# vqdang/hover_net

Measured on AMD Instinct MI355X. Metric: tiles/sec (270x270, batch 32) end-to-end incl. watershed, higher is better.
Workload: dtype fp32

## Files before the change

hover_net_amd/csrc/hvn_api.hip:

```cpp
#include <hip/hip_runtime.h>
#include <stdio.h>
#include <string.h>

#include <vector>

#include "../../include/hvn.h"
#include "hvn_kernels.h"

static thread_local char g_err[512] = "";

static int fail(int code, const char *fmt, const char *a = "", long b = 0)
{
    snprintf(g_err, sizeof(g_err), fmt, a, b);
    return code;
}

extern "C" {

int hvn_version(void) { return 104; }

#ifndef HVN_BUILD_ID
#define HVN_BUILD_ID "unstamped"
#endif
static const char hvn_build_tag[] = "hvn-build-id:" HVN_BUILD_ID;
// ... 71 lines not shown
        a.is_f32 = op->x_dtype;
        a.H = op->x.h; a.W = op->x.w;
        a.w = op->w; a.bias = op->bias;
        a.y = (float *)op->y.base;
        a.ysn = op->y.sn; a.ysy = op->y.sy; a.ysx = op->y.sx;
        a.N = batch; a.Ho = op->y.h; a.Wo = op->y.w; a.pad = op->pad_t; a.relu = op->relu; a.out_bf16 = op->act_dtype == 1;
        if (op->kh != 7 || op->kw != 7 || op->x.c != 3 || op->y.c != 64 || !op->w || !op->bias)
            return fail(HVN_E_ARG, "conv0: expects 7x7x3->64 with bias%s", "");
        if (!aligned16(a.y) || (a.ysx & 3) || (a.ysy & 3) || (a.ysn & 3)) return fail(HVN_E_ARG, "conv0: output view not 16-byte aligned%s", "");
        return hvn_launch_conv0(a, s);
    }
    case HVN_OP_CONV: {
        ConvArgs a;
        memset(&a, 0, sizeof(a));
        a.x = (const float *)op->x.base;
        a.xsn = op->x.sn; a.xsy = op->x.sy; a.xsx = op->x.sx;
        a.H = op->x.h; a.W = op->x.w; a.Cin = op->x.c;
        a.w = op->w; a.bias = op->bias;
        a.pre_s = op->pre_scale; a.pre_b = op->pre_shift;
        a.post_s = op->post_scale; a.post_b = op->post_shift;
        a.res = (const float *)op->res.base;
        a.rsn = op->res.sn; a.rsy = op->res.sy; a.rsx = op->res.sx;
        a.y = (float *)op->y.base;
        a.ysn = op->y.sn; a.ysy = op->y.sy; a.ysx = op->y.sx;
        a.N = batch; a.Ho = op->y.h; a.Wo = op->y.w; a.Cout = op->cout;
        a.KH = op->kh; a.KW = op->kw; a.stride = op->stride; a.pad_t = op->pad_t; a.pad_l = op->pad_l;
        a.relu = op->relu;
        a.groups = op->groups > 1 ? op->groups : 1;
        a.x2 = (const float *)op->x2.base;
        a.x2sn = op->x2.sn; a.x2sy = op->x2.sy; a.x2sx = op->x2.sx;
        a.Cin2 = a.x2 ? op->x2.c : 0;
        a.stride2 = op->_rsv > 0 ? op->_rsv : 1;
        if (a.x2 && (op->kh != 1 || op->kw != 1 || a.stride != 1 || a.Cin2 % 32 || !aligned16(a.x2) || ((a.x2sn | a.x2sy | a.x2sx) & 3) ||
                     a.pre_s || (long)(a.Ho - 1) * a.stride2 >= op->x2.h || (long)(a.Wo - 1) * a.stride2 >= op->x2.w))
            return fail(HVN_E_ARG, "conv: second input needs a 1x1 stride-1 op without prologue and a view that covers the output grid%s", "");
        a.M = (long)batch * a.Ho * a.Wo;
        if (!a.x || !a.w || !a.y) return fail(HVN_E_ARG, "conv: null pointer%s", "");
        if (a.Cin % 32) return fail(HVN_E_ARG, "conv: input channels must be a multiple of 32 (got %s%ld)", "", a.Cin);
        if (!aligned16(a.x) || !aligned16(a.w) || (a.xsx & 3) || (a.xsy & 3) || (a.xsn & 3))
            return fail(HVN_E_ARG, "conv: input view / weights not 16-byte aligned%s", "");
        if ((a.pre_s && !aligned16(a.pre_s)) || (a.pre_b && !aligned16(a.pre_b)) || (!a.pre_s != !a.pre_b))
            return fail(HVN_E_ARG, "conv: prologue vectors must be 16-byte aligned and come in pairs%s", "");
        if (!a.post_s != !a.post_b) return fail(HVN_E_ARG, "conv: epilogue affine must come in pairs%s", "");
        if (op->y.c != op->cout) return fail(HVN_E_ARG, "conv: output view channels != cout%s", "");
        a.nbatch = op->nbatch > 1 ? op->nbatch : 1;
        a.xb = op->batch_stride[0]; a.wb = op->batch_stride[1]; a.yb = op->batch_stride[2];
        if (a.nbatch > 1 && ((a.xb | a.wb | a.yb) & 3)) return fail(HVN_E_ARG, "conv: batch strides must keep 16-byte alignment%s", "");
        const bool bf16 = op->act_dtype == 1;
        if (bf16 && (((a.xsx | a.xsy | a.xsn) & 7) || (a.x2 && ((a.x2sx | a.x2sy | a.x2sn) & 7)) || a.nbatch > 1))
            return fail(HVN_E_ARG, "conv(bf16): input strides must be multiples of 8 elements; no batched launch%s", "");
        if (g_prof) prof_mark(s);
        const bool x3 = op->act_dtype == 2 || op->act_dtype == 3;
        if (x3 && (a.groups > 1 || (a.nbatch > 1 && (a.wb & 7)))) return fail(HVN_E_ARG, "conv(bf16x3): no grouped convs; batch stride of the planes must keep 16-byte alignment%s", "");
        int rc;
        if (bf16 && (op->tile_n == 896 || op->tile_n == 640))
            rc = hvn_launch_conv_bf16g(a, op->tile_n == 896 ? 256 : 128, s);
        else if (bf16)
            rc = hvn_launch_conv_bf16(a, op->tile_n, s);
        else if (x3 && (op->tile_n == 896 || op->tile_n == 640))
            rc = hvn_launch_conv_x3g(a, op->tile_n == 896 ? 256 : 128, op->act_dtype == 3 ? 6 : 9, s);
        else
            rc = x3 ? hvn_launch_conv_x3(a, op->tile_n, op->act_dtype == 3 ? 6 : 9, s) : hvn_launch_conv(a, op->tile_n, s);
        if (g_prof) prof_mark(s);
        if (rc) return fail(rc == -1 ? HVN_E_ARG : HVN_E_LAUNCH, "conv: launch failed (tile_n=%s%ld)", "", op->tile_n);
        return 0;
    }
    case HVN_OP_CHAIN: {
        ChainArgs a;
        memset(&a, 0, sizeof(a));
        a.x = (const float *)op->x.base;
        a.xsn = op->x.sn; a.xsy = op->x.sy; a.xsx = op->x.sx; a.K1 = op->x.c;
        a.x2 = (const float *)op->x2.base;
        a.x2sn = op->x2.sn; a.x2sy = op->x2.sy; a.x2sx = op->x2.sx;
        a.K1b = a.x2 ? op->x2.c : 0;
        a.stride2 = op->_rsv > 0 ? op->_rsv : 1;
        a.w1 = op->w;
        a.res = (const float *)op->res.base;
        a.rsn = op->res.sn; a.rsy = op->res.sy; a.rsx = op->res.sx;
        a.y = (float *)op->y.base;
        a.ysn = op->y.sn; a.ysy = op->y.sy; a.ysx = op->y.sx; a.C = op->cout;
        a.post_s = op->post_scale; a.post_b = op->post_shift;
        a.pre_s = op->pre_scale; a.pre_b = op->pre_shift;
        a.w2 = op->w2; a.bias2 = op->bias2; a.relu2 = 1;
        a.y2 = (float *)op->y2.base;
        a.y2sn = op->y2.sn; a.y2sy = op->y2.sy; a.y2sx = op->y2.sx; a.N2 = op->cout2;
        a.N = batch; a.Ho = op->y.h; a.Wo = op->y.w;
        a.M = (long)batch * a.Ho * a.Wo;
        a.bm = op->tile_n == 64 ? 64 : 128;
        const bool cx3 = op->act_dtype == 2 || op->act_dtype == 3;
        const bool cbf = op->act_dtype == 1;
        if (op->act_dtype != 0 && !cx3 && !cbf) return fail(HVN_E_ARG, "chain: act_dtype 0 (fp32), 1 (bf16) or 2 | 3 (fp32 with bf16x3 products)%s", "");
        if (cbf) {
            if (!a.x || !a.w1 || !a.y || !a.w2 || !a.y2) return fail(HVN_E_ARG, "chain: null pointer%s", "");
            if (op->kh != 1 || op->kw != 1 || op->stride != 1 || op->pad_t || op->pad_l || op->relu || op->bias)
                return fail(HVN_E_ARG, "chain: the first conv is a plain 1x1 (no bias / relu of its own)%s", "");
            if (!hvn_chain_bf16_supported(a.K1, a.K1b, a.C, a.N2) || op->y.c != a.C || op->y2.c != a.N2)
                return fail(HVN_E_ARG, "chain (bf16): needs input channels in slabs of 64 (64 or 128 in all), cout %% 256 == 0, cout2 in {64, 128} (cout2 = %s%ld)", "", a.N2);
            if (op->x.h != a.Ho || op->x.w != a.Wo || op->y2.h != a.Ho || op->y2.w != a.Wo ||
                (a.x2 && ((long)(a.Ho - 1) * a.stride2 >= op->x2.h || (long)(a.Wo - 1) * a.stride2 >= op->x2.w)))
                return fail(HVN_E_ARG, "chain: views do not cover the output grid%s", "");
            if (a.res && (a.rsn != a.ysn || a.rsy != a.ysy || a.rsx != a.ysx || op->res.c != a.C))
                return fail(HVN_E_ARG, "chain: the residual view must have the output's strides%s", "");
            if (!aligned16(a.x) || !aligned16(a.w1) || !aligned16(a.w2) || !aligned16(a.y) || !aligned16(a.y2) || (a.res && !aligned16(a.res)) ||
                (a.x2 && !aligned16(a.x2)) || ((a.xsn | a.xsy | a.xsx | a.ysn | a.ysy | a.ysx | a.y2sn | a.y2sy | a.y2sx | a.x2sn | a.x2sy | a.x2sx) & 7))
                return fail(HVN_E_ARG, "chain (bf16): views / weights not 16-byte aligned%s", "");
            if ((!a.pre_s != !a.pre_b) || (!a.post_s != !a.post_b) || (a.pre_s && (!aligned16(a.pre_s) || !aligned16(a.pre_b))) ||
                (a.post_s && (!aligned16(a.post_s) || !aligned16(a.post_b))) || (a.bias2 && !aligned16(a.bias2)))
                return fail(HVN_E_ARG, "chain: per-channel vectors must be 16-byte aligned and come in pairs%s", "");
// ... 153 lines not shown
```

hover_net_amd/csrc/hvn_kernels.h:

```cpp
#pragma once
#include <hip/hip_runtime.h>
#include <stdint.h>

#include <atomic>

static inline int hvn_max_lds_once(const void *kern, int bytes, std::atomic<unsigned long long> &done)
{
    int dev = 0;
    if (hipGetDevice(&dev) != hipSuccess) return -2;
    const unsigned long long bit = 1ull << (dev & 63);
    if (done.load(std::memory_order_acquire) & bit) return 0;
    if (hipFuncSetAttribute(kern, hipFuncAttributeMaxDynamicSharedMemorySize, bytes) != hipSuccess) return -2;
    done.fetch_or(bit, std::memory_order_release);
    return 0;
}

struct ConvArgs {
    const float *x;
    long xsn, xsy, xsx;
    int H, W, Cin;
    const float *w;
    const float *bias, *pre_s, *pre_b, *post_s, *post_b;
    const float *res;
    long rsn, rsy, rsx;
// ... 9 lines not shown
    int Cin2, stride2;
    int nbatch;
    unsigned long long *dbg;
    long xb, wb, yb;
};

int hvn_launch_conv(const ConvArgs &a, int tile_n, hipStream_t stream);

#ifndef HVN_CONV_XCD_CONTIG
#define HVN_CONV_XCD_CONTIG 1
#endif
static __device__ __forceinline__ int hvn_m_tile(int xcd, int seq_m, int groups, bool contiguous)
{
    return (HVN_CONV_XCD_CONTIG && contiguous) ? xcd * groups + seq_m : seq_m * 8 + xcd;
}

struct ChainArgs {
    const float *x;
    long xsn, xsy, xsx;
    int K1;
    const float *x2;
    long x2sn, x2sy, x2sx;
    int K1b, stride2;
    const float *w1;
    const float *res;
    long rsn, rsy, rsx;
    float *y;
    long ysn, ysy, ysx;
    int C;
    const float *post_s, *post_b, *pre_s, *pre_b;
    const float *w2;
    const float *bias2;
    int relu2;
    float *y2;
    long y2sn, y2sy, y2sx;
    int N2;
    int N, Ho, Wo;
    long M;
    int bm;
    unsigned long long *dbg;
};
int hvn_launch_conv_chain(const ChainArgs &a, hipStream_t stream);
int hvn_chain_supported(int c, int n2);
int hvn_chain_bf16_supported(int k1, int k1b, int c, int n2);
int hvn_launch_conv_chain_bf16(const ChainArgs &a, hipStream_t stream);
int hvn_launch_conv_chain_x3(const ChainArgs &a, int terms, hipStream_t stream);
int hvn_chain_x3r_supported(const ChainArgs &a);
int hvn_launch_conv_chain_x3r(const ChainArgs &a, int terms, hipStream_t stream);
int hvn_launch_conv_bf16(const ConvArgs &a, int tile_n, hipStream_t stream);
int hvn_launch_conv_bf16g(const ConvArgs &a, int bm, hipStream_t stream);
int hvn_launch_conv_x3(const ConvArgs &a, int tile_n, int terms, hipStream_t stream);
int hvn_launch_conv_x3g(const ConvArgs &a, int bm, int terms, hipStream_t stream);
int hvn_conv_x3g_supported(const ConvArgs &a, int bm);
int hvn_launch_split_x3(const float *src, uint16_t *dst, long granules, hipStream_t stream);

struct Conv0Args {
    const void *img;
    long isn, isy, isx, isc;
    int is_f32;
    int H, W;
    const float *w;
    const float *bias;
    float *y;
    long ysn, ysy, ysx;
    int N, Ho, Wo, pad;
    int relu;
    int out_bf16;
};
int hvn_launch_conv0(const Conv0Args &a, hipStream_t stream);

struct UpAddArgs {
    const float *lo;
    long lsn, lsy, lsx;
    const float *skip;
    long ssn, ssy, ssx;
    float *y;
    long ysn, ysy, ysx;
    int N, H, W, C;
    int bf16;
};
int hvn_launch_upadd(const UpAddArgs &a, hipStream_t stream);

struct HeadArgs {
    const float *x;
    long xsn, xsy, xsx;
    const float *w;
    const float *bias;
    float *y;
    int N, H, W, Cout;
    int in_bf16;
};
int hvn_launch_head(const HeadArgs &a, hipStream_t stream);

int hvn_launch_extract_patches(const uint8_t *img, int H, int W, const int32_t *coords, int P, int win, int pad_t, int pad_l, uint8_t *out,
                               hipStream_t stream);

struct PredMapArgs {
    const float *tp, *np, *hv;
    float *y;
    int N, H, W, nr_types;
};
int hvn_launch_predmap(const PredMapArgs &a, hipStream_t stream);

struct WinoArgs {
    const float *x;
    long xsn, xsy, xsx;
// ... 144 lines not shown
```

hover_net_amd/engine.py:

```python
import ctypes

import numpy as np
import torch

from . import lib as L
from . import plan as PL


def _view_struct(v, base_ptr, sn, itemsize=4):
    b = v.buf
    sx = b.c
    sy = b.w * b.c
    s = L.hvn_view()
    s.base = base_ptr + (v.y0 * sy + v.x0 * sx + v.c0) * itemsize
    s.sn, s.sy, s.sx = sn, sy, sx
    s.h, s.w, s.c, s.sc = v.h, v.w, v.c, 1
    return s


WG_SLOTS = 512
WG_SLOTS_NARROW = 768
NARROW_TILE_COST = 0.45


# ... 30 lines not shown
X3R = 128 + 0x400


def x3g_forms_for(op):
    import os

    want = os.environ.get("HVN_X3G", "1")
    if want == "0" or op.cout < 128 or int(op.extra.get("groups", 1)) != 1:
        return ()
    cin = op.x.c
    forms = []
    for code, bm, na in ((X3G_256, 256, 3), (X3G_128, 128, 2)):
        if want not in ("1", str(code)):
            continue
        if op.pre is not None and bm == 256 and na * bm * 128 + 2 * 3 * 128 * 64 + 2 * cin * 4 > 160 * 1024:
            continue
        forms.append(code)
    return tuple(forms)


def to_bf16_bits(a):
    u = np.ascontiguousarray(a, np.float32).view(np.uint32)
    return ((u + (((u >> 16) & 1) + 0x7FFF)) >> 16).astype(np.uint16)


def repack_conv_bf16(w32):
    cp, s32, taps, _ = w32.shape
    if s32 % 2:
        w32 = np.concatenate([w32, np.zeros((cp, 1, taps, 32), np.float32)], 1)
        s32 += 1
    w = w32.reshape(cp, s32 // 2, 2, taps, 32).transpose(0, 1, 3, 2, 4).reshape(cp, s32 // 2, taps, 64)
    return to_bf16_bits(w)


def split_bf16x3(w32):
    w = np.ascontiguousarray(w32, np.float32)

    def bf(a):
        bits = to_bf16_bits(a)
        return bits, (bits.astype(np.uint32) << 16).view(np.float32)

    h, hf = bf(w)
    r = w - hf
    m, mf = bf(r)
    l, _ = bf(r - mf)
    return h, m, l


def pack_conv_x3(w32):
    lead = w32.shape[:-3]
    kt = w32.shape[-3] * w32.shape[-2]
    planes = split_bf16x3(w32.reshape(lead + (kt, 32)))
    return np.stack(planes, axis=-2)


def pack_conv_x3_device(w32, device):
    w = torch.from_numpy(np.ascontiguousarray(w32, np.float32).reshape(-1, 32)).to(device)
    h = w.to(torch.bfloat16)
    r = w - h.float()
    m = r.to(torch.bfloat16)
    l = (r - m.float()).to(torch.bfloat16)
    return torch.stack((h, m, l), dim=1).view(torch.int16).reshape(-1)


class Engine:
    def __init__(self, plan, max_batch=32, device="cuda", n_split=None, dtype="fp32", n_lanes=None):
        L.require_gpu()
        assert dtype in ("fp32", "bf16")
        self.dtype = dtype
        self.isz = 4 if dtype == "fp32" else 2
        if dtype == "bf16" and any(op.kind in (PL.OP_WINO_IN, PL.OP_WINO_OUT) for op in plan.ops):
            raise ValueError("the bf16 path runs direct convolutions: build the plan with winograd=0")
        self.plan = plan
        self.max_batch = int(max_batch)
        self.device = torch.device(device)
        import os
        dflt = ("2", "2") if dtype == "fp32" else ("1", "0")
        self.n_split = int(os.environ.get("HVN_SPLIT", dflt[0])) if n_split is None else int(n_split)
        self.n_lane_streams = int(os.environ.get("HVN_LANES", dflt[1])) if n_lanes is None else int(n_lanes)
        self.split_decoder = os.environ.get("HVN_SPLIT_DECODER", "0") != "0"
        self._streams = None
        self._stream_off = 0
        self._upload_params()
        self.arena = torch.empty((self.max_batch, plan.arena_per_sample), dtype=torch.float32 if dtype == "fp32" else torch.int16,
                                 device=self.device)
        self.logits = {br: torch.empty((self.max_batch, b.c, b.h, b.w), dtype=torch.float32, device=self.device)
                       for br, b in plan.logits.items()}
        self.pred_map = None
        if plan.pred_map is not None:
            pm = plan.pred_map
            self.pred_map = torch.empty((self.max_batch, pm.h, pm.w, pm.c), dtype=torch.float32, device=self.device)
        self.ops = (L.hvn_op * len(plan.ops))()
        self._bind()
        self._sub_ops = {}
        self.tile_choice = _TILE_CACHE.setdefault(str(self.device), {})
        tile_file = os.environ.get("HVN_TILE_FILE")
        if tile_file and dtype == "fp32":
            import json
            tiles = json.load(open(tile_file))
            if len(tiles) != len(self.ops):
                raise ValueError("HVN_TILE_FILE holds %d entries for a plan of %d ops" % (len(tiles), len(self.ops)))
            for o, op, tn in zip(self.ops, plan.ops, tiles):
                if op.kind == PL.OP_CONV and ((op.tile_n == 128 and (tn in (64, 128) or (op.extra.get("x3") and tn in x3g_forms_for(op)))) or
                                              (op.tile_n == 64 and tn in (64, 320) and not op.extra.get("x3"))):
                    o.tile_n = tn
                if op.kind == PL.OP_CHAIN and (tn in (64, 128) or (tn == X3R and op.extra.get("x3"))):
                    o.tile_n = tn
        elif dtype == "fp32" and os.environ.get("HVN_TILE_SELECT", "auto") == "auto" and not os.environ.get("HVN_FORCE_TILE_N"):
            self.autotune_tiles()
        elif dtype == "bf16" and os.environ.get("HVN_TILE_SELECT", "auto") == "auto" and os.environ.get("HVN_BF16G", "1") != "0":
            self.autotune_bf16_forms()
        if os.environ.get("HVN_TILE_SELECT", "auto") == "auto" and os.environ.get("HVN_STREAM_SELECT", "1") != "0":
            self.autotune_streams()

    def _upload_params(self):
        arrays, offs, total = [], {}, 0

        def put(key, a):
            nonlocal total
            if a is None:
                return
            a = np.ascontiguousarray(a, np.float32).ravel()
            offs[key] = total
            arrays.append((total, a))
            total += (a.size + 63) // 64 * 64

        w16, off16, tot16 = [], {}, 0
        for i, op in enumerate(self.plan.ops):
            if self.dtype == "bf16" and op.kind in (PL.OP_CONV, PL.OP_CHAIN):
                wb = repack_conv_bf16(op.w).ravel()
                off16[i] = tot16
                w16.append((tot16, wb))
                tot16 += (wb.size + 127) // 128 * 128
                if op.kind == PL.OP_CHAIN:
                    wb2 = repack_conv_bf16(op.extra["w2"]).ravel()
                    off16[(i, "w2")] = tot16
                    w16.append((tot16, wb2))
                    tot16 += (wb2.size + 127) // 128 * 128
            elif self.dtype == "fp32" and op.kind in (PL.OP_CONV, PL.OP_CHAIN) and op.extra.get("x3"):
                off16[i] = tot16
                w16.append((tot16, op.w, True))
                tot16 += (3 * op.w.size + 127) // 128 * 128
                if op.kind == PL.OP_CHAIN:
                    off16[(i, "w2")] = tot16
                    w16.append((tot16, op.extra["w2"], True))
                    tot16 += (3 * op.extra["w2"].size + 127) // 128 * 128
            else:
                put((i, "w"), op.w)
            put((i, "bias"), op.bias)
            if not (op.kind == PL.OP_CHAIN and (self.dtype == "bf16" or op.extra.get("x3"))):
                put((i, "w2"), op.extra.get("w2"))
            put((i, "bias2"), op.extra.get("bias2"))
            if op.pre is not None:
                put((i, "pre_s"), op.pre[0])
                put((i, "pre_b"), op.pre[1])
            if op.post is not None:
                put((i, "post_s"), op.post[0])
                put((i, "post_b"), op.post[1])
        host = np.zeros(max(total, 64), np.float32)
        for off, a in arrays:
            host[off:off + a.size] = a
        self.params = torch.from_numpy(host).to(self.device)
        self._poff = offs
        self._poff16 = off16
        self.params16 = None
        if tot16:
            if any(len(e) == 3 for e in w16):
                self.params16 = torch.zeros(tot16, dtype=torch.int16, device=self.device)
                for off, w32, _ in w16:
                    pl = pack_conv_x3_device(w32, self.device)
                    self.params16[off:off + pl.numel()] = pl
            else:
                h16 = np.zeros(tot16, np.uint16)
                for off, a in w16:
                    h16[off:off + a.size] = a
                self.params16 = torch.from_numpy(h16.view(np.int16)).to(self.device)

    def _pptr(self, i, name):
        off = self._poff.get((i, name))
        return None if off is None else self.params.data_ptr() + 4 * off

    def _bind(self):
        P = self.plan
        abase = self.arena.data_ptr()
        sn = P.arena_per_sample
        for i, op in enumerate(P.ops):
            o = self.ops[i]
            o.act_dtype = 1 if self.dtype == "bf16" else 0
            o.kind, o.kh, o.kw, o.stride = op.kind, op.kh, op.kw, op.stride
            o.pad_t, o.pad_l, o.relu, o.cout, o.tile_n, o.x_dtype = op.pad_t, op.pad_l, op.relu, op.cout, op.tile_n, 0
            if op.kind == PL.OP_CONV and self.dtype == "fp32":
                o.tile_n = pick_tile_n(op, self.max_batch)
            o.groups = int(op.extra.get("groups", 1))
            o._rsv = int(op.extra.get("stride2", 1))
            o.nbatch = int(op.extra.get("nbatch", 1))
            for bi, bs in enumerate(op.extra.get("batch_strides", (0, 0, 0))):
                o.batch_stride[bi] = int(bs)
            if op.kind in (PL.OP_WINO_IN, PL.OP_WINO_OUT):
                o.kh, o.kw = op.extra["tiles"]
                o.stride, o._rsv = op.extra["m"], op.extra.get("r", 5)
            if op.kind == PL.OP_PREDMAP:
                o.x.base = self.logits["np"].data_ptr()
                o.res.base = self.logits["hv"].data_ptr()
                o.w = self.logits["tp"].data_ptr() if "tp" in self.logits else None
                o.cout = P.nr_types or 0
                o.y.base = self.pred_map.data_ptr()
                o.y.h, o.y.w, o.y.c = P.pred_map.h, P.pred_map.w, P.pred_map.c
                continue
            if op.kind == PL.OP_CHAIN:
                o.cout2 = int(op.extra["cout2"])
                o.w2, o.bias2 = self._pptr(i, "w2"), self._pptr(i, "bias2")
                if self.dtype == "bf16":
                    o.w2 = self.params16.data_ptr() + 2 * self._poff16[(i, "w2")]
                elif op.extra.get("x3"):
                    o.w2 = self.params16.data_ptr() + 2 * self._poff16[(i, "w2")]
                    o.act_dtype = 2 if int(op.extra["x3"]) == 9 else 3
                    o.tile_n = 128
            for fld, v in (("x", op.x), ("res", op.res), ("y", op.y), ("x2", op.extra.get("x2")), ("y2", op.extra.get("y2"))):
                if v is None:
                    continue
                if v.buf.offset >= 0:
                    setattr(o, fld, _view_struct(v, abase + self.isz * v.buf.offset, sn, self.isz))
            if op.kind == PL.OP_CONV0:
                o.x.h, o.x.w, o.x.c = op.x.h, op.x.w, 3
            if op.kind == PL.OP_HEAD:
                br = op.y.buf.name.split(".")[1]
                o.y.base = self.logits[br].data_ptr()
                o.y.h, o.y.w, o.y.c = op.y.h, op.y.w, op.y.c
            o.w = self._pptr(i, "w") if i not in self._poff16 else self.params16.data_ptr() + 2 * self._poff16[i]
            if i in self._poff16 and self.dtype == "bf16":
                o.groups = 1
            if self.dtype == "fp32" and op.kind == PL.OP_CONV and op.extra.get("x3"):
                o.act_dtype = 2 if int(op.extra["x3"]) == 9 else 3
                if o.nbatch > 1:
                    o.batch_stride[1] = int(op.w.shape[-4]) * int(op.w.shape[-3]) * int(op.w.shape[-2]) * 96
            o.bias = self._pptr(i, "bias")
            o.pre_scale, o.pre_shift = self._pptr(i, "pre_s"), self._pptr(i, "pre_b")
            o.post_scale, o.post_shift = self._pptr(i, "post_s"), self._pptr(i, "post_b")

    def autotune_streams(self, reps=3):
        split = self.n_split if (self.n_split > 1 and self.max_batch >= 2 * self.n_split) else 1
        need = (split - 1) + split * self.n_lane_streams
        if need == 0 or self.plan.ops[0].kind != PL.OP_CONV0 or not getattr(self.plan, "geo", None):
            return
        g = int(self.plan.geo.get("inp", 0))
        if g <= 0:
            return
        key = (str(self.device), split, self.n_lane_streams, self.dtype)
        if key not in _STREAM_CHOICE:
            import os
            reps = max(1, int(os.environ.get("HVN_TUNE_REPS", reps)))
            imgs = torch.zeros((self.max_batch, g, g, 3), dtype=torch.uint8, device=self.device)
            e0, e1 = torch.cuda.Event(enable_timing=True), torch.cuda.Event(enable_timing=True)
            ms = {}
            for off in range(4):
                self._stream_off, self._streams = off, None
                best = float("inf")
                for r in range(reps + 1):
                    e0.record()
                    self.run(imgs)
                    self.run(imgs)
                    e1.record()
                    e1.synchronize()
                    if r:
                        best = min(best, e0.elapsed_time(e1) / 2)
                ms[off] = best
            _STREAM_CHOICE[key] = (min(ms, key=ms.get), ms)
        self._stream_off, self._streams = _STREAM_CHOICE[key][0], None

    def autotune_tiles(self, reps=3, margin=0.985):
        import os

        lib = L.lib()
        reps = max(1, int(os.environ.get("HVN_TUNE_REPS", reps)))
        stream = torch.cuda.current_stream(self.device).cuda_stream
        e0, e1 = torch.cuda.Event(enable_timing=True), torch.cuda.Event(enable_timing=True)
        osz = ctypes.sizeof(L.hvn_op)
        base = ctypes.addressof(self.ops)

        lanes = getattr(self.plan, "lanes", None)
        enc_end = lanes[0][2] if (lanes and lanes[0][0] == "main" and len(lanes) > 1) else 0
        split = self.n_split if (self.n_split > 1 and self.max_batch >= 2 * self.n_split) else 1
        sub_n = -(-self.max_batch // split)
        if os.environ.get("HVN_TUNE_SUB", "1") == "0":
            sub_n = self.max_batch

        def time_op(i):
            best = float("inf")
# ... 277 lines not shown
```

hover_net_amd/lib.py:

```python
import ctypes
import os
import subprocess

_HERE = os.path.dirname(os.path.abspath(__file__))
LIB_PATH = os.path.join(_HERE, "libhvn_hip.so")
VARIANTS = {
    "pad": ("-DHVN_SWZ=0",),
    "noxcd": ("-DHVN_WINO_XCD=0", "-DHVN_CONV_XCD_CONTIG=0"),
    "fullepi": ("-DHVN_X3G_FULL_EPI=1",),
    "wn1": ("-DHVN_X3G_WN=1",),
    "prev": (),
    "trace": ("-DHVN_TRACE_FINE=1",),
}
CSRC = os.path.join(_HERE, "csrc")
SOURCES = ("hvn_conv.hip", "hvn_conv_chain.hip", "hvn_conv_chain_x3.hip", "hvn_conv_chain_x3r.hip", "hvn_conv_bf16.hip", "hvn_conv_bf16g.hip", "hvn_conv_chain_bf16.hip", "hvn_conv_x3.hip", "hvn_conv_x3g.hip", "hvn_net_ops.hip", "hvn_postproc.hip", "hvn_api.hip", "hvn_train.hip", "hvn_wgrad_x3.hip", "hvn_targets.hip", "hvn_wsi_merge.hip",
           "hvn_augment.hip", "hvn_train_api.hip", "hvn_contour.cpp", "hvn_metrics.hip")
HIPCC_FLAGS = ("--offload-arch=gfx950", "-O3", "-std=c++17", "-fPIC", "-shared", "-ffp-contract=off",
               "-fvisibility=hidden", "-Wno-unused-value", "-pthread")


class hvn_view(ctypes.Structure):
    _fields_ = [("base", ctypes.c_void_p), ("sn", ctypes.c_int64), ("sy", ctypes.c_int64), ("sx", ctypes.c_int64),
                ("h", ctypes.c_int32), ("w", ctypes.c_int32), ("c", ctypes.c_int32), ("sc", ctypes.c_int32)]


class hvn_op(ctypes.Structure):
    _fields_ = [(k, ctypes.c_int32) for k in ("kind", "kh", "kw", "stride", "pad_t", "pad_l", "relu", "cout", "tile_n", "x_dtype", "groups", "_rsv")] + \
               [("x", hvn_view), ("res", hvn_view), ("y", hvn_view), ("x2", hvn_view)] + \
               [(k, ctypes.c_void_p) for k in ("w", "bias", "pre_scale", "pre_shift", "post_scale", "post_shift")] + \
               [("batch_stride", ctypes.c_int64 * 3), ("nbatch", ctypes.c_int32), ("act_dtype", ctypes.c_int32)] + \
               [("y2", hvn_view), ("w2", ctypes.c_void_p), ("bias2", ctypes.c_void_p), ("cout2", ctypes.c_int32), ("_rsv2", ctypes.c_int32)]


class hvn_top(ctypes.Structure):
    _fields_ = [(k, ctypes.c_int32) for k in ("kind", "kh", "kw", "stride", "pad_t", "pad_l", "groups", "cout", "cin_g", "mode", "lead_pad", "_pad")] + \
               [("x", hvn_view), ("y", hvn_view), ("dx", hvn_view), ("dy", hvn_view), ("p", ctypes.c_void_p * 6),
                ("eps", ctypes.c_float), ("momentum", ctypes.c_float), ("net", ctypes.POINTER(hvn_op)),
                ("batch_stride", ctypes.c_int64 * 3), ("nbatch", ctypes.c_int32), ("_pad2", ctypes.c_int32)]


class hvn_pack_desc(ctypes.Structure):
    _fields_ = [("src", ctypes.c_void_p), ("dst", ctypes.c_void_p)] + [(k, ctypes.c_int32) for k in ("cout", "cin_g", "groups", "taps", "mode", "lead_pad")] + \
               [("gmat", ctypes.c_void_p)]


class hvn_loss(ctypes.Structure):
    _fields_ = [(k, ctypes.c_void_p) for k in ("logits_np", "logits_hv", "logits_tp", "true_np", "true_tp", "true_hv",
                                               "grad_np", "grad_hv", "grad_tp", "sums", "sobel_ws")] + \
               [(k, ctypes.c_int32) for k in ("n", "h", "w", "nr_types")] + [("total_pixels", ctypes.c_double), ("weight", ctypes.c_float * 6),
                                                                             ("partials", ctypes.c_void_p), ("partials_cap", ctypes.c_int64)]


class hvn_inst_rec(ctypes.Structure):
    _fields_ = [("label", ctypes.c_int32), ("area", ctypes.c_int32), ("rmin", ctypes.c_int32), ("rmax", ctypes.c_int32),
                ("cmin", ctypes.c_int32), ("cmax", ctypes.c_int32), ("sum_x", ctypes.c_double), ("sum_y", ctypes.c_double),
                ("type", ctypes.c_int32), ("type_count", ctypes.c_int32)]


EXPORTS = (
    "hvn_version", "hvn_build_id", "hvn_last_error", "hvn_device_ok", "hvn_run_plan", "hvn_run_op", "hvn_profile_enable",
    "hvn_profile_conv_ms", "hvn_profile_conv_launches", "hvn_profile_conv_ms_list", "hvn_postproc_workspace_bytes", "hvn_postproc",
    "hvn_postproc_taps", "hvn_postproc_stats", "hvn_instance_table_workspace_bytes", "hvn_instance_table", "hvn_trace_contours",
    "hvn_run_train_plan", "hvn_run_train_plan_ws", "hvn_train_workspace_bytes", "hvn_train_last_error", "hvn_loss_partials_count", "hvn_loss_forward", "hvn_loss_backward", "hvn_adam_step",
    "hvn_extract_patches", "hvn_gen_targets", "hvn_gen_targets_workspace_bytes", "hvn_augment_shape", "hvn_augment_input",
    "hvn_wsi_merge_normal", "hvn_wsi_merge_fixing",
    "hvn_pair_table_workspace_bytes", "hvn_pair_table", "hvn_label_range", "hvn_remap_label_workspace_bytes", "hvn_remap_label",
    "hvn_label_areas", "hvn_label_permute",
)
# ... 194 lines not shown
```

hover_net_amd/plan.py:

```python
from dataclasses import dataclass, field

import numpy as np

from . import arch

OP_CONV0, OP_CONV, OP_UPADD, OP_HEAD, OP_PREDMAP, OP_WINO_IN, OP_WINO_OUT, OP_CHAIN = 1, 2, 3, 4, 5, 6, 7, 8


@dataclass
class Buf:
    name: str
    h: int
    w: int
    c: int
    dtype: str = "f32"
    offset: int = -1
    first: int = 10 ** 9
    last: int = -1

    @property
    def size(self):
        return self.h * self.w * self.c


# ... 181 lines not shown
                relu=relu, cout=cout, tile_n=tn)
        op.bias = None if b is None else np.asarray(b, np.float32)
        op.pre = None if pre is None else (np.asarray(pre[0], np.float32), np.asarray(pre[1], np.float32))
        op.post = None if post is None else (np.asarray(post[0], np.float32), np.asarray(post[1], np.float32))
        op.extra["cin_real"] = (x.c + (x2.c if x2 is not None else 0)) // groups
        op.extra["groups"] = groups
        if x2 is not None:
            assert y.h == (x2.h - 1) // stride2 + 1
            op.extra["x2"], op.extra["stride2"] = x2, stride2
            if x2.buf.dtype == "f32":
                op.extra["reads"] = [x2.buf]
        return self.add(op)

    def conv_winograd(self, name, x, y, wt, *, pad=(0, 0), bn=None, relu=0, share_in=False, m=4):
        from . import winograd as WG

        cout, cin, kh, kw = wt.shape
        assert kh == kw and (kh, m) in ((5, 2), (5, 4), (5, 6), (3, 4), (3, 6)) and x.c == cin and y.c == cout
        r = kh
        assert y.h == x.h + pad[0] + pad[1] - (r - 1)
        if m == 6 and -(-y.h // 6) * -(-y.w // 6) < 64:
            m = 4
        at, _g, bt = WG.mats(m, r)
        n2 = (m + r - 1) ** 2
        s = b = None
        if bn is not None:
            s, b = bn
            wt = wt * s[:, None, None, None]
        ty, tx = -(-y.h // m), -(-y.w // m)
        t1 = ty * tx
        key = (id(x.buf), x.y0, x.x0, x.h, x.w, x.c0, x.c, pad[0], m, r)
        cache = self.__dict__.setdefault("_wino_in", {})
        if key not in cache:
            vbuf = self.buf(name + ".V", n2, t1, cin)
            op = Op(OP_WINO_IN, name + ".wino_in", x=x, y=View(vbuf), w=np.ascontiguousarray(bt, np.float32),
                    pad_t=pad[0], pad_l=pad[0], extra={"tiles": (ty, tx), "shared": share_in, "m": m, "r": r})
            self.add(op)
            cache[key] = vbuf
        vbuf = cache[key]
        mbuf = self.buf(name + ".M", n2, t1, cout)
        tn = _tile_n(cout)
        cout_pad = (cout + tn - 1) // tn * tn
        packed = _wino_packed(wt, m, n2, cout, cin, cout_pad)
        g = Op(OP_CONV, name + ".wino_gemm", x=View(vbuf, 0, 0, 1, t1), y=View(mbuf, 0, 0, 1, t1), w=packed, cout=cout, tile_n=tn)
        g.extra.update(nbatch=n2, batch_strides=(t1 * cin, cout_pad * cin, t1 * cout), cin_real=cin, groups=1,
                       algo_flops=2.0 * y.h * y.w * cout * cin * r * r, exec_flops=2.0 * n2 * t1 * cout * cin)
        self.add(g)
        for bb in (vbuf, mbuf):
            bb.last = max(bb.last, len(self.ops) - 1)
        o = Op(OP_WINO_OUT, name + ".wino_out", x=View(mbuf), y=y, w=np.ascontiguousarray(at, np.float32),
               bias=None if b is None else np.asarray(b, np.float32), relu=relu, cout=cout, extra={"tiles": (ty, tx), "m": m, "r": r})
        return self.add(o)

    def mark_x3(self, terms, d1=True, chain="d0"):
        import re

        assert terms in (9, 6), terms
        for op in self.ops:
            if op.kind != OP_CONV or int(op.extra.get("groups", 1)) != 1 or op.tile_n not in (128, 64):
                continue
            seam = False
            if re.match(r"^d0\.units\.\d+\.conv[13]$", op.name) or op.name == "d1.units.0.conv1":
                if not chain or op.name == "d0.units.0.conv1":
                    continue
                seam = True
            if re.match(r"^d1\.units\.\d+\.conv[13]$", op.name) and op.name != "d1.units.0.conv1":
                if not d1:
                    continue
                seam = chain == "d0d1"
            op.extra["x3"] = terms
            if seam:
                op.extra["x3_chain"] = True

    def reindex(self):
        ops, self.ops = self.ops, []
        for b in self.bufs:
            b.first, b.last = 10 ** 9, -1
        for op in ops:
            self.add(op)

    def fuse_chains(self, max_n2=128, accept=None):
        out, i, ops = [], 0, self.ops
        while i < len(ops):
            a = ops[i]
            b = ops[i + 1] if i + 1 < len(ops) else None

            def plain1x1(o):
                return (o is not None and o.kind == OP_CONV and o.kh == 1 and o.kw == 1 and o.stride == 1 and o.pad_t == 0 and
                        not o.extra.get("nbatch") and o.extra.get("groups", 1) == 1 and (not o.extra.get("x3") or o.extra.get("x3_chain")))

            ok = (plain1x1(a) and plain1x1(b) and int(a.extra.get("x3", 0)) == int(b.extra.get("x3", 0)) and (a.res is not None or a.extra.get("x2") is not None) and a.pre is None and
                  a.bias is None and not a.relu and a.cout % 64 == 0 and a.x.c + (a.extra["x2"].c if a.extra.get("x2") is not None else 0) >= 64 and
                  b.res is None and b.extra.get("x2") is None and b.post is None and b.relu == 1 and
                  b.cout in (64, 128) and b.cout <= max_n2 and
                  (b.x.buf is a.y.buf and (b.x.y0, b.x.x0, b.x.h, b.x.w, b.x.c0, b.x.c) == (a.y.y0, a.y.x0, a.y.h, a.y.w, a.y.c0, a.y.c)) and
                  (b.y.h, b.y.w) == (a.y.h, a.y.w) and
                  (a.res is None or (a.res.buf.w, a.res.buf.c, a.res.h, a.res.w, a.res.c) == (a.y.buf.w, a.y.buf.c, a.y.h, a.y.w, a.y.c)))
            if ok and accept is not None and not accept(a, b):
                ok = False
            if not ok:
                out.append(a)
                i += 1
                continue
            op = Op(OP_CHAIN, a.name + "+" + b.name.split(".", 1)[1] if b.name.split(".")[0] == a.name.split(".")[0] else a.name + "+" + b.name,
                    x=a.x, y=a.y, res=a.res, w=a.w, post=a.post, pre=b.pre, cout=a.cout, tile_n=0)
            op.extra.update(cin_real=a.extra["cin_real"], groups=1, cout2=b.cout, w2=b.w, bias2=b.bias, y2=b.y, parts=(a, b))
            if a.extra.get("x3"):
                op.extra["x3"] = int(a.extra["x3"])
            if a.extra.get("x2") is not None:
                op.extra.update(x2=a.extra["x2"], stride2=a.extra["stride2"], reads=a.extra.get("reads", []))
            out.append(op)
# ... 113 lines not shown
    u3in = View(P.buf("u3.in", d_sz[2], d_sz[2], 1024))
    P.add(Op(OP_UPADD, "u3.upadd", x=d3, res=skips[2], y=u3in))
    d1c = skips[1].crop(g["crop1"])
    d0c = skips[0].crop(g["crop0"])
    cm = (k - 1) // 2
    heads = {}
    for br in arch.branch_names(nr_types):
        pb = "decoder.%s." % br
        cur_in = u3in
        for uname, cmid, units, cat_sz, skip in (("u3", 256, 8, g["u3_cat"], d1c), ("u2", 128, 4, g["u2_cat"], d0c)):
            p = pb + uname + "."
            ctot = cmid + units * arch.DENSE_GROWTH
            cat = View(P.buf(p + "cat", cat_sz, cat_sz, ctot))
            if winograd and (k == 5 or wino3):
                P.conv_winograd(p + "conva", cur_in, cat.chans(0, cmid), W(p + "conva.weight"), share_in=(uname == "u3"),
                                m=wino_stage.get(uname, wino_m) if k == 5 else wino3_m)
            else:
                P.conv(p + "conva", cur_in, cat.chans(0, cmid), W(p + "conva.weight"))
            c = cmid
            win = cat
            for i in range(units):
                q = p + "dense.units.%d." % i
                t1 = View(P.buf(q + "t1", win.h, win.w, arch.DENSE_MID))
                P.conv(q + "conv1", win.chans(0, c), t1, W(q + "conv1.weight"), bn=BN(q + "conv1/bn"), relu=1,
                       pre=BN(q + "preact_bna/bn"))
                win = win.crop(cm)
                P.conv(q + "conv2", t1, win.chans(c, arch.DENSE_GROWTH), W(q + "conv2.weight"), groups=arch.DENSE_GROUPS)
                c += arch.DENSE_GROWTH
            uo = View(P.buf(p + "out", win.h, win.w, ctot))
            P.conv(p + "convf", win.chans(0, ctot), uo, W(p + "convf.weight"), pre=BN(p + "dense.blk_bna.bn"))
            nxt = View(P.buf(p + "up", 2 * win.h, 2 * win.w, ctot))
            P.add(Op(OP_UPADD, p + "upadd", x=uo, res=skip, y=nxt))
            cur_in = nxt
        u1 = View(P.buf(pb + "u1", g["out"], g["out"], 64))
        if winograd and (k == 5 or wino3):
            P.conv_winograd(pb + "u1.conva", cur_in, u1, W(pb + "u1.conva.weight"), pad=_tf_same(cur_in.h, k, 1),
                            bn=BN(pb + "u0.bn"), relu=1, m=wino_stage.get("u1", wino_m) if k == 5 else wino3_m)
        else:
            P.conv(pb + "u1.conva", cur_in, u1, W(pb + "u1.conva.weight"), pad=_tf_same(cur_in.h, k, 1),
                   bn=BN(pb + "u0.bn"), relu=1)
        oc = arch.branch_out_ch(br, nr_types)
        lg = Buf("logits." + br, g["out"], g["out"], oc)
        P.logits[br] = lg
        heads[br] = P.add(Op(OP_HEAD, pb + "u0.conv", x=u1, y=View(lg),
                             w=np.ascontiguousarray(W(pb + "u0.conv.weight").reshape(oc, 64), np.float32),
                             bias=np.asarray(W(pb + "u0.conv.bias"), np.float32), cout=oc))
    if with_predmap:
        pm = Buf("pred_map", g["out"], g["out"], 3 if nr_types is None else 4)
        P.pred_map = pm
        P.add(Op(OP_PREDMAP, "infer_step.epilogue", y=View(pm), extra={"branches": list(arch.branch_names(nr_types))}))
    if x3 is None:
        x3 = 9 if conservative else int(os.environ.get("HVN_X3", "6"))
    if x3:
        P.mark_x3(int(x3), d1=os.environ.get("HVN_X3_D1", "1") != "0", chain=os.environ.get("HVN_X3_CHAIN", "d0"))
    if isinstance(chain, str) and chain.startswith("bf16"):
        blocks = tuple(chain.split(":", 1)[1].replace("d0d1", "d0,d1").split(",")) if ":" in chain else ("d0", "d1")

        def bf16_seam(a, b):
            x2 = a.extra.get("x2")
            ka = a.x.c + (x2.c if x2 is not None else 0)
            return a.name.split(".")[0] in blocks and a.x.c % 64 == 0 and (x2 is None or x2.c % 64 == 0) and ka in (64, 128) and a.cout % 256 == 0
        P.fuse_chains(128, accept=bf16_seam)
    elif chain:
        P.fuse_chains(int(os.environ.get("HVN_CHAIN_MAXN2", "128")))
    if os.environ.get("HVN_FUSE_UPADD", "0") != "0":
        P.fuse_upadd_into_winograd()
    lanes, cur, start = [], None, 0
    for i, op in enumerate(P.ops):
        lane = op.name.split(".")[1] if (op.name.startswith("decoder.") and not op.extra.get("shared")) else "main"
        if lane != cur:
            if cur is not None:
                lanes.append((cur, start, i))
            cur, start = lane, i
    lanes.append((cur, start, len(P.ops)))
    br = [(lo, hi) for lane, lo, hi in lanes if lane != "main"]
    if br:
        r0, r1 = br[0][0], br[-1][1] - 1
        for b in P.bufs:
            if b.last >= r0 and b.first <= r1:
                b.first, b.last = min(b.first, r0), max(b.last, r1)
    P.pack()
    P.lanes = lanes
    return P
```

Measured before the change: 757.6.

## Add split-bf16x3 MFMA kernel for grouped 5x5 dense-unit convs

Adds a dedicated kernel for the decoder dense-unit 5x5 grouped convolutions (4 groups, 128->32 channels). Inputs are split into bf16 hi/mid/lo planes in LDS and run through MFMA 16x16x32 bf16 instructions with 6 or 9 cross terms. Weights are prepacked on the host into a dx-interleaved table. The kernel streams row tiles down each column, prefetching the next rows into registers while computing the current ones. This replaces the generic fp32 grouped conv path and trades exact fp32 accumulation for split-bf16 accuracy. It is enabled by default unless conservative mode is set.

```diff
diff --git a/hover_net_amd/csrc/hvn_api.hip b/hover_net_amd/csrc/hvn_api.hip
--- a/hover_net_amd/csrc/hvn_api.hip
+++ b/hover_net_amd/csrc/hvn_api.hip
@@ -147,8 +147,11 @@
         if (g_prof) prof_mark(s);
         const bool x3 = op->act_dtype == 2 || op->act_dtype == 3;
         if (x3 && (a.groups > 1 || (a.nbatch > 1 && (a.wb & 7)))) return fail(HVN_E_ARG, "conv(bf16x3): no grouped convs; batch stride of the planes must keep 16-byte alignment%s", "");
+        const bool x3d = op->act_dtype == 4 || op->act_dtype == 5;
         int rc;
-        if (bf16 && (op->tile_n == 896 || op->tile_n == 640))
+        if (x3d)
+            rc = hvn_launch_dense_grouped_x3(a, op->act_dtype == 4 ? 9 : 6, s);
+        else if (bf16 && (op->tile_n == 896 || op->tile_n == 640))
             rc = hvn_launch_conv_bf16g(a, op->tile_n == 896 ? 256 : 128, s);
         else if (bf16)
             rc = hvn_launch_conv_bf16(a, op->tile_n, s);
diff --git a/hover_net_amd/csrc/hvn_dense_x3.hip b/hover_net_amd/csrc/hvn_dense_x3.hip
--- /dev/null
+++ b/hover_net_amd/csrc/hvn_dense_x3.hip
@@ -0,0 +1,174 @@
+#include "hvn_conv_common.h"
+
+#define DX_TH 8
+#define DX_TW 64
+#define DX_PH (DX_TH + 4)
+#define DX_PW (DX_TW + 4)
+#define DX_QS ((DX_PH * DX_PW) | 1)
+#define DX_LDS (3 * 4 * DX_QS * 16)
+#define DX_NT 256
+#define DX_CUS 256
+#define DX_S0 7
+#define DX_S1 9
+static_assert(2 * DX_S0 * DX_NT >= DX_PH * DX_PW * 4 && DX_S1 * DX_NT >= DX_TH * DX_PW * 4, "staging passes");
+
+template <int NTERMS>
+__global__ __launch_bounds__(DX_NT, 1) void hvn_dense_grouped_x3(const ConvArgs p, int tiles_x, int tiles_y, int run, int runs)
+{
+    extern __shared__ __attribute__((aligned(16))) unsigned char dx_patch[];
+    const int tid = threadIdx.x, lane = tid & 63, wave = tid >> 6;
+    const int l15 = lane & 15, q = lane >> 4;
+    int bid = blockIdx.x;
+    const int g = bid & 3;
+    bid >>= 2;
+    const int tx = bid % tiles_x;
+    bid /= tiles_x;
+    const int rn = bid % runs;
+    const int n = bid / runs;
+    const int ty0 = rn * run, ty1 = min(ty0 + run, tiles_y);
+    const int ox0 = tx * DX_TW;
+    const int chalf = wave & 1, r0 = 4 * (wave >> 1);
+    const bool active = ox0 + 32 * chalf < p.Wo;
+    const int co = l15 & 7, dx = l15 >> 3;
+    const uint16_t *wtab = (const uint16_t *)p.w + (long)g * (6 * 5 * 3 * 512) + 8 * lane;
+    auto load_b = [&](int tc, bf16x8 (&b)[5][3]) {
+#pragma unroll
+        for (int tr = 0; tr < 5; ++tr)
+#pragma unroll
+            for (int pl = 0; pl < 3; ++pl)
+                b[tr][pl] = __builtin_bit_cast(bf16x8, *(const u32x4 *)(wtab + ((tc * 5 + tr) * 3 + pl) * 512));
+    };
+    const float *xin = p.x + (long)n * p.xsn + 32 * g;
+    const bool narrow = p.Wo - ox0 <= 32;
+    const int pw = narrow ? 36 : DX_PW;
+    auto fetch = [&](int i, int row0, int items, f32x4 &v0, f32x4 &v1) {
+        const int px_i = i >> 2, oc = i & 3;
+        const int py = narrow ? px_i / 36 : px_i / DX_PW;
+        const int iy = row0 + py, ix = ox0 + px_i - py * pw;
+        v0 = v1 = (f32x4){0.f, 0.f, 0.f, 0.f};
+        if (i < items && iy < p.H && ix < p.W) {
+            const float *src = xin + (long)iy * p.xsy + (long)ix * p.xsx + 8 * oc;
+            v0 = *(const f32x4 *)src;
+            v1 = *(const f32x4 *)(src + 4);
+        }
+    };
+    auto park = [&](int i, int row0, int items, const f32x4 &v0, const f32x4 &v1) {
+        if (i < items) {
+            const int px_i = i >> 2, oc = i & 3;
+            const int py = narrow ? px_i / 36 : px_i / DX_PW;
+            const int px = px_i - py * pw;
+            bf16x8 h, m, l;
+            hvn_split3x8(v0, v1, h, m, l);
+            unsigned char *dst = dx_patch + (oc * DX_QS + ((row0 + py) % DX_PH) * DX_PW + px) * 16;
+            *(bf16x8 *)(dst) = h;
+            *(bf16x8 *)(dst + 4 * DX_QS * 16) = m;
+            *(bf16x8 *)(dst + 8 * DX_QS * 16) = l;
+        }
+    };
+    bf16x8 wb[2][5][3];
+    load_b(0, wb[0]);
+    __builtin_amdgcn_sched_barrier(0);
+    {
+        const int row0 = ty0 * DX_TH, items = DX_PH * pw * 4;
+        for (int i0 = tid; i0 < items; i0 += DX_S0 * DX_NT) {
+            f32x4 v0[DX_S0], v1[DX_S0];
+#pragma unroll
+            for (int j = 0; j < DX_S0; ++j) fetch(i0 + DX_NT * j, row0, items, v0[j], v1[j]);
+            __builtin_amdgcn_sched_barrier(0);
+#pragma unroll
+            for (int j = 0; j < DX_S0; ++j) park(i0 + DX_NT * j, row0, items, v0[j], v1[j]);
+        }
+    }
+    const float bias = p.bias ? p.bias[8 * g + co] : 0.f;
+    const float lo = p.relu ? 0.f : -__builtin_inff();
+    const unsigned char *acol = dx_patch + (q * DX_QS + 32 * chalf + 2 * l15) * 16;
+    __syncthreads();
+    for (int ty = ty0; ty < ty1; ++ty) {
+        const int oy0 = ty * DX_TH;
+        const bool more = ty + 1 < ty1;
+        const int nrow0 = oy0 + DX_PH, nitems = more ? DX_TH * pw * 4 : 0;
+        f32x4 n0[DX_S1], n1[DX_S1];
+#pragma unroll
+        for (int j = 0; j < DX_S1; ++j) fetch(tid + DX_NT * j, nrow0, nitems, n0[j], n1[j]);
+        __builtin_amdgcn_sched_barrier(0);
+        if (active) {
+            int arow[8];
+#pragma unroll
+            for (int pr = 0; pr < 8; ++pr) arow[pr] = ((oy0 + r0 + pr) % DX_PH) * (DX_PW * 16);
+            f32x4 acc[4];
+#pragma unroll
+            for (int r = 0; r < 4; ++r) acc[r] = (f32x4){0.f, 0.f, 0.f, 0.f};
+#pragma unroll
+            for (int tc = 0; tc < 6; ++tc) {
+                load_b(tc + 1 < 6 ? tc + 1 : 0, wb[(tc + 1) & 1]);
+                __builtin_amdgcn_sched_barrier(0);
+#pragma unroll
+                for (int pr = 0; pr < 8; ++pr) {
+                    bf16x8 a[3];
+#pragma unroll
+                    for (int pl = 0; pl < 3; ++pl)
+                        a[pl] = __builtin_bit_cast(bf16x8, *(const u32x4 *)(acol + arow[pr] + (pl * 4 * DX_QS + tc) * 16));
+#pragma unroll
+                    for (int s = 4; s >= 0; --s) {
+                        if (NTERMS == 6 && s > 2) continue;
+#pragma unroll
+                        for (int pa = 2; pa >= 0; --pa) {
+                            const int pb = s - pa;
+                            if (pb < 0 || pb > 2) continue;
+#pragma unroll
+                            for (int tr = 0; tr < 5; ++tr) {
+                                const int r = pr - tr;
+                                if (r < 0 || r > 3) continue;
+                                acc[r] = __builtin_amdgcn_mfma_f32_16x16x32_bf16(a[pa], wb[tc & 1][tr][pb], acc[r], 0, 0, 0);
+                            }
+                        }
+                    }
+                }
+            }
+#pragma unroll
+            for (int r = 0; r < 4; ++r) {
+                const int oy = oy0 + r0 + r;
+#pragma unroll
+                for (int i = 0; i < 4; ++i) {
+                    const int ox = ox0 + 32 * chalf + 2 * (4 * q + i) + dx;
+                    if (oy < p.Ho && ox < p.Wo)
+                        p.y[(long)n * p.ysn + (long)oy * p.ysy + (long)ox * p.ysx + 8 * g + co] = fmaxf(acc[r][i] + bias, lo);
+                }
+            }
+        }
+        if (more) {
+            __syncthreads();
+#pragma unroll
+            for (int j = 0; j < DX_S1; ++j) park(tid + DX_NT * j, nrow0, nitems, n0[j], n1[j]);
+            __syncthreads();
+        }
+    }
+}
+
+template <int NTERMS>
+static int launch_dense_x3(const ConvArgs &a, hipStream_t stream)
+{
+    const int tiles_x = (a.Wo + DX_TW - 1) / DX_TW, tiles_y = (a.Ho + DX_TH - 1) / DX_TH;
+    const long cols = 4L * tiles_x * a.N;
+    int runs = (int)((DX_CUS + cols - 1) / cols);
+    runs = runs < 1 ? 1 : (runs > tiles_y ? tiles_y : runs);
+    const int run = (tiles_y + runs - 1) / runs;
+    runs = (tiles_y + run - 1) / run;
+    static std::atomic<unsigned long long> attr_done{0};
+    auto kern = hvn_dense_grouped_x3<NTERMS>;
+    if (hvn_max_lds_once((const void *)kern, DX_LDS, attr_done)) return -2;
+    const long grid = cols * runs;
+    if (grid <= 0 || grid > 0x7fffffffL) return -1;
+    hipLaunchKernelGGL(kern, dim3((unsigned)grid), dim3(DX_NT), DX_LDS, stream, a, tiles_x, tiles_y, run, runs);
+    return hipGetLastError() == hipSuccess ? 0 : -2;
+}
+
+int hvn_launch_dense_grouped_x3(const ConvArgs &a, int terms, hipStream_t stream)
+{
+    if (a.groups != 4 || a.Cin != 128 || a.Cout != 32 || a.stride != 1 || hvn_conv_padded(a) || a.pre_s || a.res || a.post_s || a.x2 ||
+        a.nbatch > 1 || a.KH != 5 || a.KW != 5 || a.N <= 0 || a.Ho <= 0 || a.Wo <= 0 || a.Ho + 4 > a.H || a.Wo + 4 > a.W)
+        return -1;
+    if (terms == 9) return launch_dense_x3<9>(a, stream);
+    if (terms == 6) return launch_dense_x3<6>(a, stream);
+    return -1;
+}
diff --git a/hover_net_amd/csrc/hvn_kernels.h b/hover_net_amd/csrc/hvn_kernels.h
--- a/hover_net_amd/csrc/hvn_kernels.h
+++ b/hover_net_amd/csrc/hvn_kernels.h
@@ -85,6 +85,7 @@
 int hvn_launch_conv_x3(const ConvArgs &a, int tile_n, int terms, hipStream_t stream);
 int hvn_launch_conv_x3g(const ConvArgs &a, int bm, int terms, hipStream_t stream);
 int hvn_conv_x3g_supported(const ConvArgs &a, int bm);
+int hvn_launch_dense_grouped_x3(const ConvArgs &a, int terms, hipStream_t stream);
 int hvn_launch_split_x3(const float *src, uint16_t *dst, long granules, hipStream_t stream);
 
 struct Conv0Args {
diff --git a/hover_net_amd/engine.py b/hover_net_amd/engine.py
--- a/hover_net_amd/engine.py
+++ b/hover_net_amd/engine.py
@@ -106,6 +106,19 @@
     kt = w32.shape[-3] * w32.shape[-2]
     planes = split_bf16x3(w32.reshape(lead + (kt, 32)))
     return np.stack(planes, axis=-2)
+
+
+def pack_dense_x3(w32):
+    w = np.ascontiguousarray(w32, np.float32)
+    assert w.shape == (32, 4, 25, 32), w.shape
+    tab = np.zeros((4, 6, 5, 4, 2, 8, 8), np.float32)
+    for g in range(4):
+        blk = w[8 * g:8 * g + 8, g].reshape(8, 5, 5, 4, 8)
+        for dx in range(2):
+            for c in range(5):
+                tab[g, c + dx, :, :, dx] = blk[:, :, c].transpose(1, 2, 0, 3)
+    planes = split_bf16x3(tab.reshape(4, 6, 5, 512))
+    return np.ascontiguousarray(np.stack(planes, axis=3)).ravel()
 
 
 def pack_conv_x3_device(w32, device):
@@ -191,6 +204,11 @@
                     off16[(i, "w2")] = tot16
                     w16.append((tot16, wb2))
                     tot16 += (wb2.size + 127) // 128 * 128
+            elif self.dtype == "fp32" and op.kind == PL.OP_CONV and op.extra.get("x3_dense"):
+                wb = pack_dense_x3(op.w)
+                off16[i] = tot16
+                w16.append((tot16, wb))
+                tot16 += (wb.size + 127) // 128 * 128
             elif self.dtype == "fp32" and op.kind in (PL.OP_CONV, PL.OP_CHAIN) and op.extra.get("x3"):
                 off16[i] = tot16
                 w16.append((tot16, op.w, True))
@@ -221,8 +239,9 @@
         if tot16:
             if any(len(e) == 3 for e in w16):
                 self.params16 = torch.zeros(tot16, dtype=torch.int16, device=self.device)
-                for off, w32, _ in w16:
-                    pl = pack_conv_x3_device(w32, self.device)
+                for e in w16:
+                    off, w32 = e[0], e[1]
+                    pl = pack_conv_x3_device(w32, self.device) if len(e) == 3 else torch.from_numpy(w32.view(np.int16)).to(self.device)
                     self.params16[off:off + pl.numel()] = pl
             else:
                 h16 = np.zeros(tot16, np.uint16)
@@ -288,6 +307,8 @@
                 o.act_dtype = 2 if int(op.extra["x3"]) == 9 else 3
                 if o.nbatch > 1:
                     o.batch_stride[1] = int(op.w.shape[-4]) * int(op.w.shape[-3]) * int(op.w.shape[-2]) * 96
+            if self.dtype == "fp32" and op.kind == PL.OP_CONV and op.extra.get("x3_dense"):
+                o.act_dtype = 4 if int(op.extra["x3_dense"]) == 9 else 5
             o.bias = self._pptr(i, "bias")
             o.pre_scale, o.pre_shift = self._pptr(i, "pre_s"), self._pptr(i, "pre_b")
             o.post_scale, o.post_shift = self._pptr(i, "post_s"), self._pptr(i, "post_b")
diff --git a/hover_net_amd/lib.py b/hover_net_amd/lib.py
--- a/hover_net_amd/lib.py
+++ b/hover_net_amd/lib.py
@@ -13,7 +13,7 @@
     "trace": ("-DHVN_TRACE_FINE=1",),
 }
 CSRC = os.path.join(_HERE, "csrc")
-SOURCES = ("hvn_conv.hip", "hvn_conv_chain.hip", "hvn_conv_chain_x3.hip", "hvn_conv_chain_x3r.hip", "hvn_conv_bf16.hip", "hvn_conv_bf16g.hip", "hvn_conv_chain_bf16.hip", "hvn_conv_x3.hip", "hvn_conv_x3g.hip", "hvn_net_ops.hip", "hvn_postproc.hip", "hvn_api.hip", "hvn_train.hip", "hvn_wgrad_x3.hip", "hvn_targets.hip", "hvn_wsi_merge.hip",
+SOURCES = ("hvn_conv.hip", "hvn_conv_chain.hip", "hvn_conv_chain_x3.hip", "hvn_conv_chain_x3r.hip", "hvn_conv_bf16.hip", "hvn_conv_bf16g.hip", "hvn_conv_chain_bf16.hip", "hvn_conv_x3.hip", "hvn_conv_x3g.hip", "hvn_dense_x3.hip", "hvn_net_ops.hip", "hvn_postproc.hip", "hvn_api.hip", "hvn_train.hip", "hvn_wgrad_x3.hip", "hvn_targets.hip", "hvn_wsi_merge.hip",
            "hvn_augment.hip", "hvn_train_api.hip", "hvn_contour.cpp", "hvn_metrics.hip")
 HIPCC_FLAGS = ("--offload-arch=gfx950", "-O3", "-std=c++17", "-fPIC", "-shared", "-ffp-contract=off",
                "-fvisibility=hidden", "-Wno-unused-value", "-pthread")
diff --git a/hover_net_amd/plan.py b/hover_net_amd/plan.py
--- a/hover_net_amd/plan.py
+++ b/hover_net_amd/plan.py
@@ -257,11 +257,15 @@
                bias=None if b is None else np.asarray(b, np.float32), relu=relu, cout=cout, extra={"tiles": (ty, tx), "m": m, "r": r})
         return self.add(o)
 
-    def mark_x3(self, terms, d1=True, chain="d0"):
+    def mark_x3(self, terms, d1=True, chain="d0", dense=False):
         import re
 
         assert terms in (9, 6), terms
         for op in self.ops:
+            if (dense and op.kind == OP_CONV and re.search(r"\.dense\.units\.\d+\.conv2$", op.name) and int(op.extra.get("groups", 1)) == 4 and
+                    op.x.c == 128 and op.cout == 32 and op.kh == 5 and op.kw == 5 and op.stride == 1 and op.pad_t == 0 and op.pad_l == 0 and
+                    op.pre is None and op.post is None and op.res is None):
+                op.extra["x3_dense"] = terms
             if op.kind != OP_CONV or int(op.extra.get("groups", 1)) != 1 or op.tile_n not in (128, 64):
                 continue
             seam = False
@@ -481,7 +485,8 @@
     if x3 is None:
         x3 = 9 if conservative else int(os.environ.get("HVN_X3", "6"))
     if x3:
-        P.mark_x3(int(x3), d1=os.environ.get("HVN_X3_D1", "1") != "0", chain=os.environ.get("HVN_X3_CHAIN", "d0"))
+        P.mark_x3(int(x3), d1=os.environ.get("HVN_X3_D1", "1") != "0", chain=os.environ.get("HVN_X3_CHAIN", "d0"),
+                  dense=not conservative and os.environ.get("HVN_X3_DENSE", "1") != "0")
     if isinstance(chain, str) and chain.startswith("bf16"):
         blocks = tuple(chain.split(":", 1)[1].replace("d0d1", "d0,d1").split(",")) if ":" in chain else ("d0", "d1")
 
```

New measurement: 770.4, median of 6. 1.7% higher.
